# azrael417/mlperf-deepcam

Hardware: AMD Instinct MI355X
Metric: samples/sec (768x1152x16) train step (higher is better)
Workload: dtype bf16; 1 GPU; DeepLabV3+/Xception train step (fwd + weighted CE + bwd + LAMB), 768x1152x16, local_batch=8, bf16 activations / fp32 master weights, random-init seed 333; local_batch=8, global_batch=8, parallelism=dp1, optimizer=LAMB, hip_graph=False, launch_list_replay=False

## Files before the change

### mlperf-deepcam_amd/csrc/dwtile_s2.hip

```cpp
#include "dwtile.h"
#include "dwtile_common.h"
#include "mfma_tile.h"

namespace dc {

namespace {

static __device__ __attribute__((aligned(256))) unsigned char dws2_zero_page[256];

template <int CG, int TH_>
struct S2Cfg {
  static constexpr int TH = TH_, TW = 8 * (32 / CG);
  static constexpr int NSL = 128 / CG;
  static constexpr int SPR = TW / DT_PX;
  static constexpr int SPT = TH * SPR / NSL;
  static_assert(SPT * NSL == TH * SPR, "tile does not divide into strips");
};
constexpr int lds_bytes(int hh, int hw, int cg) { return (hh * hw * cg + 255) / 256 * 256 * 16; }

template <typename T, int HH, int HW, int CG>
__device__ inline void stage_tile(char* smem, const T* __restrict__ in, int ldin, int n, int iy0, int ix0, int cg0, int ngroups, int H,
                                  int W) {
  constexpr int KPV = Elem<T>::kPerVec;
  constexpr int HP = HH * HW, ITER = (HP * CG + 255) / 256;
  const int tid = threadIdx.x;
  const int wv = __builtin_amdgcn_readfirstlane(tid >> 6);
  const int g = tid % CG;
  const bool gok = cg0 + g < ngroups;
  const T* base = in + (size_t)n * H * W * ldin + (size_t)(cg0 + g) * KPV;
#pragma unroll
  for (int it = 0; it < ITER; ++it) {
    const int hp = (it * 256 + tid) / CG;
    const int hy = hp / HW, hx = hp - hy * HW;
    const int iy = iy0 + hy, ix = ix0 + hx;
    const bool ok = gok && hp < HP && (unsigned)iy < (unsigned)H && (unsigned)ix < (unsigned)W;
    const void* src = ok ? (const void*)(base + ((size_t)iy * W + ix) * ldin) : (const void*)dws2_zero_page;
    __builtin_amdgcn_global_load_lds((gas_ptr)src, (lds_ptr)(smem + (it * 256 + wv * 64) * 16), 16, 0, 0);
  }
}

struct S2Args {
  int Hi, Wi, Ho, Wo, C, ncgb, ntx, nty;
  const float* pscale;
  const float* pshift;
  int prelu;
};

template <typename T, int CG>
__global__ __launch_bounds__(256) void dws2_fwd_kernel(const T* __restrict__ in, int ldin, const float* __restrict__ wp,
                                                       T* __restrict__ out, int ldout, S2Args a) {
  typedef S2Cfg<CG, 4> K;
  constexpr int KPV = Elem<T>::kPerVec, KH = KPV / 2;
  constexpr int HH = 2 * K::TH + 1, HW = 2 * K::TW + 1, WC = 2 * DT_PX + 1;
  extern __shared__ __attribute__((aligned(16))) char smem[];
  const int t = xcd_remap(blockIdx.x, gridDim.x);
  const int cgb = t % a.ncgb;
  int r = t / a.ncgb;
  const int tx = r % a.ntx;
  r /= a.ntx;
  const int ty = r % a.nty, n = r / a.nty;
  const int ngroups = a.C / KPV;
  const int cg0 = cgb * CG, y0 = ty * K::TH, x0 = tx * K::TW;
  stage_tile<T, HH, HW, CG>(smem, in, ldin, n, 2 * y0 - 1, 2 * x0 - 1, cg0, ngroups, a.Hi, a.Wi);
  const int h = threadIdx.x % (2 * CG), sl = threadIdx.x / (2 * CG);
  const bool cok = cg0 + (h >> 1) < ngroups;
  const int ch0 = cok ? cg0 * KPV + h * KH : 0;
  float wk[9][KH];
  load_taps<KH>(wp, ch0, a.C, false, wk);
  __syncthreads();
  if (a.pscale != nullptr) {
    bn_transform_tile<T, HH, HW, CG>(smem, 2 * y0 - 1, 2 * x0 - 1, a.Hi, a.Wi, a.pscale, a.pshift, a.prelu, cg0, ngroups);
    __syncthreads();
  }
  if (!cok) return;
  const char* tile = smem + h * 8;
#pragma unroll 1
  for (int k = 0; k < K::SPT; ++k) {
    const int q = sl + K::NSL * k;
    const int row = q / K::SPR, xs = (q % K::SPR) * DT_PX;
    float acc[DT_PX][KH];
#pragma unroll
    for (int j = 0; j < DT_PX; ++j)
#pragma unroll
      for (int e = 0; e < KH; ++e) acc[j][e] = 0.f;
#pragma unroll
    for (int ky = 0; ky < 3; ++ky)
#pragma unroll
      for (int c = 0; c < WC; ++c) {
        float f[KH];
        unpack8(*reinterpret_cast<const vec8*>(tile + ((2 * row + ky) * HW + 2 * xs + c) * (CG * 16)), f, T());
#pragma unroll
        for (int kx = 0; kx < 3; ++kx) {
          if ((c - kx) >= 0 && ((c - kx) & 1) == 0 && (c - kx) / 2 < DT_PX) {
#pragma unroll
            for (int e = 0; e < KH; ++e) acc[(c - kx) / 2][e] = fmaf(f[e], wk[ky * 3 + kx][e], acc[(c - kx) / 2][e]);
          }
        }
      }
    const int oy = y0 + row;
    if (oy < a.Ho) {
#pragma unroll
      for (int j = 0; j < DT_PX; ++j) {
        const int ox = x0 + xs + j;
        if (ox < a.Wo) {
          vec8 v;
          pack8(v, acc[j], T());
          *reinterpret_cast<vec8*>(out + (((size_t)n * a.Ho + oy) * a.Wo + ox) * ldout + ch0) = v;
        }
      }
    }
  }
}

template <typename T, int CG, bool WG>
__global__ __launch_bounds__(256) void dws2_dgrad_kernel(const T* __restrict__ dy, int lddy, const float* __restrict__ wp,
                                                         const T* __restrict__ addend, int ldadd, T* __restrict__ dx, int lddx, S2Args a,
                                                         const DwBnStats st, int ntiles, int tpb) {
  typedef S2Cfg<CG, 8> K;
  constexpr int KPV = Elem<T>::kPerVec, KH = KPV / 2;
  constexpr int HH = K::TH / 2 + 1, HW = K::TW / 2 + 1;
  extern __shared__ __attribute__((aligned(16))) char smem[];
  const int t = xcd_remap(blockIdx.x, gridDim.x);
  const int cgb = t % a.ncgb;
  const int srow = t / a.ncgb;
  const int ngroups = a.C / KPV;
  const int cg0 = cgb * CG;
  const int h = threadIdx.x % (2 * CG), sl = threadIdx.x / (2 * CG);
  const bool cok = cg0 + (h >> 1) < ngroups;
  const int ch0 = cok ? cg0 * KPV + h * KH : 0;
  float wk[9][KH];
  load_taps<KH>(wp, ch0, a.C, false, wk);
  const bool stats = st.slab != nullptr;
  BnAcc<KH> bn;
  if (stats) bn.init(st, ch0);
  else if (WG) bn.init_affine(st, ch0);
  float dwa[WG ? 9 : 1][KH];
#pragma unroll
  for (int t9 = 0; t9 < (WG ? 9 : 1); ++t9)
#pragma unroll
    for (int e = 0; e < KH; ++e) dwa[t9][e] = 0.f;
  const char* tile = smem + h * 8;
  const int tbeg = srow * tpb, tend = min(ntiles, tbeg + tpb);
  for (int ti = tbeg; ti < tend; ++ti) {
    const int tx = ti % a.ntx;
    int r = ti / a.ntx;
    const int ty = r % a.nty, n = r / a.nty;
    const int y0 = ty * K::TH, x0 = tx * K::TW;
    if (ti != tbeg) __syncthreads();
    stage_tile<T, HH, HW, CG>(smem, dy, lddy, n, y0 / 2, x0 / 2, cg0, ngroups, a.Ho, a.Wo);
    auto load_y = [&](int k, vec8 (&yv)[DT_PX]) {
      const int q = sl + K::NSL * k;
      const int iy = y0 + q / K::SPR, xs = (q % K::SPR) * DT_PX;
#pragma unroll
      for (int j = 0; j < DT_PX; ++j) {
        const int ix = x0 + xs + j;
        vec8 z;
        z.w[0] = z.w[1] = 0u;
        yv[j] = (iy < a.Hi && ix < a.Wi) ? *reinterpret_cast<const vec8*>(reinterpret_cast<const T*>(st.y) + (((size_t)n * a.Hi + iy) * a.Wi + ix) * st.ldy + ch0) : z;
      }
    };
    vec8 yv[DT_PX], ynext[DT_PX];
    if (cok && (stats || WG)) load_y(0, yv);
    __syncthreads();
#pragma unroll 1
    for (int k = 0; k < (cok ? K::SPT : 0); ++k) {
      const int q = sl + K::NSL * k;
      const int row = q / K::SPR, xs = (q % K::SPR) * DT_PX;
      const int iy = y0 + row;
      if ((stats || WG) && k + 1 < K::SPT) load_y(k + 1, ynext);
      vec8 av[DT_PX];
      if (addend != nullptr) {
#pragma unroll
        for (int j = 0; j < DT_PX; ++j) {
          const int ix = x0 + xs + j;
          vec8 z;
          z.w[0] = z.w[1] = 0u;
          av[j] = (iy < a.Hi && ix < a.Wi) ? *reinterpret_cast<const vec8*>(addend + (((size_t)n * a.Hi + iy) * a.Wi + ix) * ldadd + ch0) : z;
        }
      }
      float acc[DT_PX][KH];
#pragma unroll
      for (int j = 0; j < DT_PX; ++j)
#pragma unroll
        for (int e = 0; e < KH; ++e) acc[j][e] = 0.f;
      float xh[WG ? DT_PX : 1][KH];
      if constexpr (WG) {
#pragma unroll
        for (int j = 0; j < DT_PX; ++j) {
          const bool in = iy < a.Hi && x0 + xs + j < a.Wi;
          float yf[KH];
          unpack8(yv[j], yf, T());
#pragma unroll
          for (int e = 0; e < KH; ++e) {
            const float v = fmaf(yf[e], bn.ms[e], bn.mh[e]);
            yf[e] = st.relu ? fmaxf(v, 0.f) : v;
          }
          vec8 rr;
          pack8(rr, yf, T());
          unpack8(rr, xh[j], T());
          if (!in) {
#pragma unroll
            for (int e = 0; e < KH; ++e) xh[j][e] = 0.f;
          }
        }
      }
#pragma unroll
      for (int ky = 0; ky < 3; ++ky) {
        const int num = row + 1 - ky;
        const bool yfit = (num & 1) == 0;
        const int trow = yfit ? num >> 1 : 0;
#pragma unroll
        for (int j = 0; j < DT_PX; ++j)
#pragma unroll
          for (int kx = 0; kx < 3; ++kx) {
            if (((j + 1 - kx) & 1) == 0) {
              const int tcol = (xs + j + 1 - kx) / 2;
              float f[KH];
              unpack8(*reinterpret_cast<const vec8*>(tile + (trow * HW + tcol) * (CG * 16)), f, T());
#pragma unroll
              for (int e = 0; e < KH; ++e) {
                const float fv = yfit ? f[e] : 0.f;
                acc[j][e] = fmaf(fv, wk[ky * 3 + kx][e], acc[j][e]);
                if constexpr (WG) dwa[ky * 3 + kx][e] = fmaf(fv, xh[j][e], dwa[ky * 3 + kx][e]);
              }
            }
          }
      }
      if (iy < a.Hi) {
#pragma unroll
        for (int j = 0; j < DT_PX; ++j) {
          const int ix = x0 + xs + j;
          if (ix < a.Wi) {
            if (addend != nullptr) {
              float ad[KH];
              unpack8(av[j], ad, T());
#pragma unroll
              for (int e = 0; e < KH; ++e) acc[j][e] += ad[e];
            }
            vec8 v;
            pack8(v, acc[j], T());
            *reinterpret_cast<vec8*>(dx + (((size_t)n * a.Hi + iy) * a.Wi + ix) * lddx + ch0) = v;
            if (stats) {
              float gs[KH], yf[KH];
              unpack8(v, gs, T());
              unpack8(yv[j], yf, T());
              bn.add(gs, yf, st.relu);
            }
          }
        }
      }
#pragma unroll
      for (int j = 0; j < DT_PX; ++j) yv[j] = ynext[j];
    }
  }
  if (stats) {
    __syncthreads();
    bn_acc_store<KH, K::NSL, CG * KPV>(reinterpret_cast<float*>(smem), bn.a, bn.b, cok, h, sl, st, srow, cg0 * KPV, a.C);
  }
  if constexpr (WG) {
    __syncthreads();
    float* red = reinterpret_cast<float*>(smem);
    constexpr int CW = CG * KPV;
    if (cok) {
#pragma unroll
      for (int tp = 0; tp < 9; ++tp)
#pragma unroll
        for (int e = 0; e < KH; ++e) red[(sl * 9 + tp) * CW + h * KH + e] = dwa[tp][e];
    }
    __syncthreads();
    for (int i = threadIdx.x; i < 9 * CW; i += 256) {
      const int tp = i / CW, cl = i % CW;
      const int c = cg0 * KPV + cl;
      if (c < a.C) {
        float s = 0.f;
#pragma unroll
        for (int q = 0; q < K::NSL; ++q) s += red[(q * 9 + tp) * CW + cl];
        st.wslab[((size_t)srow * 9 + tp) * a.C + c] = s;
      }
    }
  }
}

template <typename T, int CG>
__global__ __launch_bounds__(256) void dws2_wgrad_kernel(const T* __restrict__ x, int ldx, const T* __restrict__ dy, int lddy,
                                                         float* __restrict__ slab, S2Args a, int ntiles, int tpb) {
  typedef S2Cfg<CG, 4> K;
  constexpr int KPV = Elem<T>::kPerVec, KH = KPV / 2;
  constexpr int HH = 2 * K::TH + 1, HW = 2 * K::TW + 1, WC = 2 * DT_PX + 1;
  extern __shared__ __attribute__((aligned(16))) char smem[];
  const int t = xcd_remap(blockIdx.x, gridDim.x);
  const int cgb = t % a.ncgb, srow = t / a.ncgb;
  const int ngroups = a.C / KPV;
  const int cg0 = cgb * CG;
  const int h = threadIdx.x % (2 * CG), sl = threadIdx.x / (2 * CG);
  const bool cok = cg0 + (h >> 1) < ngroups;
  const int ch0 = cok ? cg0 * KPV + h * KH : 0;
  float acc[9][KH];
#pragma unroll
  for (int tp = 0; tp < 9; ++tp)
#pragma unroll
    for (int e = 0; e < KH; ++e) acc[tp][e] = 0.f;
  const int tbeg = srow * tpb, tend = min(ntiles, tbeg + tpb);
  const char* tile = smem + h * 8;
  for (int ti = tbeg; ti < tend; ++ti) {
    const int tx = ti % a.ntx;
    int r = ti / a.ntx;
    const int ty = r % a.nty, n = r / a.nty;
    const int y0 = ty * K::TH, x0 = tx * K::TW;
    if (ti != tbeg) __syncthreads();
    stage_tile<T, HH, HW, CG>(smem, x, ldx, n, 2 * y0 - 1, 2 * x0 - 1, cg0, ngroups, a.Hi, a.Wi);
    auto load_dy = [&](int k, vec8 (&gv)[DT_PX]) {
      const int q = sl + K::NSL * k;
      const int row = q / K::SPR, xs = (q % K::SPR) * DT_PX;
      const int oy = y0 + row;
#pragma unroll
      for (int j = 0; j < DT_PX; ++j) {
        const int ox = x0 + xs + j;
        const bool ok = cok && oy < a.Ho && ox < a.Wo;
        vec8 z;
        z.w[0] = z.w[1] = 0u;
        gv[j] = ok ? *reinterpret_cast<const vec8*>(dy + (((size_t)n * a.Ho + oy) * a.Wo + ox) * lddy + ch0) : z;
      }
    };
    vec8 gcur[DT_PX], gnext[DT_PX];
    load_dy(0, gcur);
    __syncthreads();
    if (a.pscale != nullptr) {
      bn_transform_tile<T, HH, HW, CG>(smem, 2 * y0 - 1, 2 * x0 - 1, a.Hi, a.Wi, a.pscale, a.pshift, a.prelu, cg0, ngroups);
      __syncthreads();
    }
    if (cok) {
#pragma unroll 1
      for (int k = 0; k < K::SPT; ++k) {
        if (k + 1 < K::SPT) load_dy(k + 1, gnext);
        const int q = sl + K::NSL * k;
        const int row = q / K::SPR, xs = (q % K::SPR) * DT_PX;
        float gf[DT_PX][KH];
#pragma unroll
        for (int j = 0; j < DT_PX; ++j) unpack8(gcur[j], gf[j], T());
#pragma unroll
        for (int ky = 0; ky < 3; ++ky)
#pragma unroll
          for (int c = 0; c < WC; ++c) {
            float f[KH];
            unpack8(*reinterpret_cast<const vec8*>(tile + ((2 * row + ky) * HW + 2 * xs + c) * (CG * 16)), f, T());
#pragma unroll
            for (int kx = 0; kx < 3; ++kx) {
              if ((c - kx) >= 0 && ((c - kx) & 1) == 0 && (c - kx) / 2 < DT_PX) {
#pragma unroll
                for (int e = 0; e < KH; ++e) acc[ky * 3 + kx][e] = fmaf(gf[(c - kx) / 2][e], f[e], acc[ky * 3 + kx][e]);
              }
            }
          }
#pragma unroll
        for (int j = 0; j < DT_PX; ++j) gcur[j] = gnext[j];
      }
    }
  }
  __syncthreads();
  float* red = reinterpret_cast<float*>(smem);
  constexpr int CW = CG * KPV;
#pragma unroll
  for (int tp = 0; tp < 9; ++tp)
#pragma unroll
    for (int e = 0; e < KH; ++e) red[(sl * 9 + tp) * CW + h * KH + e] = acc[tp][e];
  __syncthreads();
  for (int i = threadIdx.x; i < 9 * CW; i += 256) {
    const int tp = i / CW, cl = i % CW;
    const int c = cg0 * KPV + cl;
    if (c < a.C) {
      float s = 0.f;
#pragma unroll
      for (int q = 0; q < K::NSL; ++q) s += red[(q * 9 + tp) * CW + cl];
      slab[((size_t)srow * 9 + tp) * a.C + c] = s;
    }
  }
}

static int pick_cg(int ngroups) { return ngroups <= 8 ? 8 : ngroups <= 16 ? 16 : 32; }

constexpr int S2_DGRAD_WGS = 1024;
static int s2_dgrad_plan(int kpv, int C, int N, int Hi, int Wi, int* tpb_out) {
  const int cg = pick_cg(C / kpv);
  const int ntiles = N * cdiv(Hi, 8) * cdiv(Wi, 8 * (32 / cg));
  const int ncgb = cdiv(C / kpv, cg);
  int tpb = cdiv((long)ntiles * ncgb, S2_DGRAD_WGS);
  if (tpb < 1) tpb = 1;
  if (tpb_out) *tpb_out = tpb;
  return cdiv(ntiles, tpb);
}

template <typename T, int CG>
static void launch3(int mode, S2Args a, int N, const void* p0, int ld0, const float* wp, const void* p1, int ld1, void* out, int ldout,
                    float* slab, int* rows_out, hipStream_t st, DwBnStats bs) {
  constexpr int TW = 8 * (32 / CG);
  constexpr int LDS_F = lds_bytes(9, 2 * TW + 1, CG);
  constexpr int LDS_D0 = lds_bytes(5, TW / 2 + 1, CG);
  constexpr int FOLD2 = (128 / CG) * 2 * CG * Elem<T>::kPerVec * (int)sizeof(float);
  constexpr int LDS_D = LDS_D0 > FOLD2 ? LDS_D0 : FOLD2;
  constexpr int FOLD = (128 / CG) * 9 * CG * Elem<T>::kPerVec * (int)sizeof(float);
  a.ntx = cdiv(mode == 1 ? a.Wi : a.Wo, TW);
  a.nty = cdiv(mode == 1 ? a.Hi : a.Ho, mode == 1 ? 8 : 4);
  a.ncgb = cdiv(a.C / Elem<T>::kPerVec, CG);
  const int ntiles = N * a.ntx * a.nty;
  if (mode == 0) {
    DC_ONCE((void)hipFuncSetAttribute(reinterpret_cast<const void*>(&dws2_fwd_kernel<T, CG>), hipFuncAttributeMaxDynamicSharedMemorySize, LDS_F));
    hipLaunchKernelGGL((dws2_fwd_kernel<T, CG>), dim3(ntiles * a.ncgb), dim3(256), LDS_F, st, (const T*)p0, ld0, wp, (T*)out, ldout, a);
  } else if (mode == 1) {
    int tpb = 1;
    const int rows = s2_dgrad_plan(Elem<T>::kPerVec, a.C, N, a.Hi, a.Wi, &tpb);
    bs.rows = rows;
    if (rows_out) *rows_out = rows;
    if (bs.wslab != nullptr) {
      constexpr int LDS_DW = LDS_D > FOLD ? LDS_D : FOLD;
      DC_ONCE((void)hipFuncSetAttribute(reinterpret_cast<const void*>(&dws2_dgrad_kernel<T, CG, true>), hipFuncAttributeMaxDynamicSharedMemorySize, LDS_DW));
      hipLaunchKernelGGL((dws2_dgrad_kernel<T, CG, true>), dim3(rows * a.ncgb), dim3(256), LDS_DW, st, (const T*)p0, ld0, wp, (const T*)p1, ld1, (T*)out, ldout, a, bs, ntiles, tpb);
    } else {
      DC_ONCE((void)hipFuncSetAttribute(reinterpret_cast<const void*>(&dws2_dgrad_kernel<T, CG, false>), hipFuncAttributeMaxDynamicSharedMemorySize, LDS_D));
      hipLaunchKernelGGL((dws2_dgrad_kernel<T, CG, false>), dim3(rows * a.ncgb), dim3(256), LDS_D, st, (const T*)p0, ld0, wp, (const T*)p1, ld1, (T*)out, ldout, a, bs, ntiles, tpb);
    }
  } else {
    constexpr int LDS_W = LDS_F > FOLD ? LDS_F : FOLD;
    DC_ONCE((void)hipFuncSetAttribute(reinterpret_cast<const void*>(&dws2_wgrad_kernel<T, CG>), hipFuncAttributeMaxDynamicSharedMemorySize, LDS_W));
    long tpb = ((long)ntiles * a.ncgb + 256) / 512;
    if (tpb < 1) tpb = 1;
    while (cdiv(ntiles, tpb) > DWT_MAX_ROWS) ++tpb;
    const int rows = cdiv(ntiles, tpb);
    *rows_out = rows;
    hipLaunchKernelGGL((dws2_wgrad_kernel<T, CG>), dim3(rows * a.ncgb), dim3(256), LDS_W, st, (const T*)p0, ld0, (const T*)p1, ld1, slab, a, ntiles, (int)tpb);
  }
}

template <typename T>
static void launch2(int mode, const S2Args& a, int N, const void* p0, int ld0, const float* wp, const void* p1, int ld1, void* out,
                    int ldout, float* slab, int* rows_out, hipStream_t st, const DwBnStats& bs) {
  const int cg = pick_cg(a.C / Elem<T>::kPerVec);
  if (cg == 32) launch3<T, 32>(mode, a, N, p0, ld0, wp, p1, ld1, out, ldout, slab, rows_out, st, bs);
  else if (cg == 16) launch3<T, 16>(mode, a, N, p0, ld0, wp, p1, ld1, out, ldout, slab, rows_out, st, bs);
  else launch3<T, 8>(mode, a, N, p0, ld0, wp, p1, ld1, out, ldout, slab, rows_out, st, bs);
}

}

int launch_dw_tile_s2(int dtype, int mode, int N, int Hi, int Wi, int C, const void* p0, int ld0, const float* wp, const void* p1, int ld1,
                      void* out, int ldout, float* slab, int* rows_out, hipStream_t st, const float* pscale, const float* pshift, int prelu,
                      const DwBnStats* bnstats) {
  DwBnStats bs;
  if (bnstats != nullptr && mode == 1) bs = *bnstats; else { bs.slab = nullptr; bs.y = nullptr; bs.ldy = 0; bs.mean = bs.invstd = bs.mscale = bs.mshift = nullptr; bs.relu = 0; bs.rows = 0; bs.wslab = nullptr; }
  S2Args a;
  a.pscale = mode == 1 ? nullptr : pscale; a.pshift = pshift; a.prelu = prelu;
  a.Hi = Hi; a.Wi = Wi; a.Ho = (Hi - 1) / 2 + 1; a.Wo = (Wi - 1) / 2 + 1; a.C = C;
  a.ncgb = a.ntx = a.nty = 0;
  DC_REQUIRE((long)N * Hi * Wi < (1L << 31), "dc_dwconv: tensor too large for the tiled stride-2 path");
  int rows = 0;
  if (dtype == DC_BF16) launch2<bf16>(mode, a, N, p0, ld0, wp, p1, ld1, out, ldout, slab, &rows, st, bs);
  else launch2<float>(mode, a, N, p0, ld0, wp, p1, ld1, out, ldout, slab, &rows, st, bs);
  if (rows_out) *rows_out = rows;
  DC_LAUNCHED(mode == 0 ? "dw_tile_s2_fwd" : mode == 1 ? "dw_tile_s2_dgrad" : "dw_tile_s2_wgrad");
  return 0;
}

int dw_tile_s2_dgrad_rows(int dtype, int C, int N, int Hi, int Wi) { return s2_dgrad_plan(dtype == DC_BF16 ? 8 : 4, C, N, Hi, Wi, nullptr); }

}
```

Before: 269.8 samples/s.

## Double-buffer stride-2 depthwise dgrad tiles and specialize on row parity

```diff
diff --git a/mlperf-deepcam_amd/csrc/dwtile_s2.hip b/mlperf-deepcam_amd/csrc/dwtile_s2.hip
--- a/mlperf-deepcam_amd/csrc/dwtile_s2.hip
+++ b/mlperf-deepcam_amd/csrc/dwtile_s2.hip
@@ -112,13 +112,24 @@
   }
 }
 
-template <typename T, int CG, bool WG>
-__global__ __launch_bounds__(256) void dws2_dgrad_kernel(const T* __restrict__ dy, int lddy, const float* __restrict__ wp,
-                                                         const T* __restrict__ addend, int ldadd, T* __restrict__ dx, int lddx, S2Args a,
-                                                         const DwBnStats st, int ntiles, int tpb) {
+__device__ inline vec8 load8_if(const void* p, bool ok) {
+  vec8 v;
+  v.w[0] = v.w[1] = 0u;
+  if (ok) v = *reinterpret_cast<const vec8*>(p);
+  return v;
+}
+
+template <typename T, int CG, bool WG, bool ST>
+__global__ __launch_bounds__(256, 3) void dws2_dgrad_kernel(const T* __restrict__ dy, int lddy, const float* __restrict__ wp,
+                                                            const T* __restrict__ addend, int ldadd, T* __restrict__ dx, int lddx, S2Args a,
+                                                            const DwBnStats st, int ntiles, int tpb) {
   typedef S2Cfg<CG, 8> K;
   constexpr int KPV = Elem<T>::kPerVec, KH = KPV / 2;
   constexpr int HH = K::TH / 2 + 1, HW = K::TW / 2 + 1;
+  constexpr int TILE_B = lds_bytes(HH, HW, CG);
+  constexpr int RS = K::NSL / K::SPR;
+  static_assert(K::NSL % K::SPR == 0 && RS % 2 == 0, "the row parity of a thread's strips must not depend on the strip");
+  static_assert((2 * CG * K::SPR) % 64 == 0, "the row parity must be the same for the lanes of a wave");
   extern __shared__ __attribute__((aligned(16))) char smem[];
   const int t = xcd_remap(blockIdx.x, gridDim.x);
   const int cgb = t % a.ncgb;
@@ -128,118 +139,117 @@
   const int h = threadIdx.x % (2 * CG), sl = threadIdx.x / (2 * CG);
   const bool cok = cg0 + (h >> 1) < ngroups;
   const int ch0 = cok ? cg0 * KPV + h * KH : 0;
-  float wk[9][KH];
-  load_taps<KH>(wp, ch0, a.C, false, wk);
-  const bool stats = st.slab != nullptr;
+  const int r0 = sl / K::SPR, xs = (sl % K::SPR) * DT_PX;
+  const int par = __builtin_amdgcn_readfirstlane(r0 & 1);
+  constexpr bool stats = ST, needy = ST || WG;
+  const bool add = !ST && addend != nullptr;
   BnAcc<KH> bn;
   if (stats) bn.init(st, ch0);
   else if (WG) bn.init_affine(st, ch0);
-  float dwa[WG ? 9 : 1][KH];
-#pragma unroll
-  for (int t9 = 0; t9 < (WG ? 9 : 1); ++t9)
-#pragma unroll
-    for (int e = 0; e < KH; ++e) dwa[t9][e] = 0.f;
-  const char* tile = smem + h * 8;
+  float dwa[WG ? 6 : 1][KH];
+#pragma unroll
+  for (int t6 = 0; t6 < (WG ? 6 : 1); ++t6)
+#pragma unroll
+    for (int e = 0; e < KH; ++e) dwa[t6][e] = 0.f;
   const int tbeg = srow * tpb, tend = min(ntiles, tbeg + tpb);
-  for (int ti = tbeg; ti < tend; ++ti) {
-    const int tx = ti % a.ntx;
-    int r = ti / a.ntx;
-    const int ty = r % a.nty, n = r / a.nty;
-    const int y0 = ty * K::TH, x0 = tx * K::TW;
-    if (ti != tbeg) __syncthreads();
+
+  auto tiles = [&](auto par_tag) {
+    constexpr int PAR = decltype(par_tag)::value;
+    constexpr int NL = PAR ? 2 : 1;
+    float wl[3 * NL][KH];
+#pragma unroll
+    for (int l = 0; l < NL; ++l)
+#pragma unroll
+      for (int kx = 0; kx < 3; ++kx)
+#pragma unroll
+        for (int e = 0; e < KH; ++e) wl[l * 3 + kx][e] = wp[(size_t)((PAR ? 2 * l : 1) * 3 + kx) * a.C + ch0 + e];
+    auto coords = [&](int ti, int& n, int& y0, int& x0) {
+      const int r = ti / a.ntx;
+      x0 = (ti - r * a.ntx) * K::TW;
+      n = r / a.nty;
+      y0 = (r - n * a.nty) * K::TH;
+    };
+    auto pixel = [&](int n, int iy) { return ((unsigned)n * a.Hi + iy) * a.Wi; };
+    int n, y0, x0;
+    coords(tbeg, n, y0, x0);
     stage_tile<T, HH, HW, CG>(smem, dy, lddy, n, y0 / 2, x0 / 2, cg0, ngroups, a.Ho, a.Wo);
-    auto load_y = [&](int k, vec8 (&yv)[DT_PX]) {
-      const int q = sl + K::NSL * k;
-      const int iy = y0 + q / K::SPR, xs = (q % K::SPR) * DT_PX;
+    vec8 yv[DT_PX], av[DT_PX];
+    if (cok) {
+      const unsigned p = pixel(n, y0 + r0) + x0 + xs;
 #pragma unroll
       for (int j = 0; j < DT_PX; ++j) {
-        const int ix = x0 + xs + j;
-        vec8 z;
-        z.w[0] = z.w[1] = 0u;
-        yv[j] = (iy < a.Hi && ix < a.Wi) ? *reinterpret_cast<const vec8*>(reinterpret_cast<const T*>(st.y) + (((size_t)n * a.Hi + iy) * a.Wi + ix) * st.ldy + ch0) : z;
-      }
-    };
-    vec8 yv[DT_PX], ynext[DT_PX];
-    if (cok && (stats || WG)) load_y(0, yv);
-    __syncthreads();
+        const bool ok = y0 + r0 < a.Hi && x0 + xs + j < a.Wi;
+        if (needy) yv[j] = load8_if(reinterpret_cast<const T*>(st.y) + (size_t)(p + j) * st.ldy + ch0, ok);
+        if (add) av[j] = load8_if(addend + (size_t)(p + j) * ldadd + ch0, ok);
+      }
+    }
+    for (int ti = tbeg; ti < tend; ++ti) {
+      const char* tile = smem + ((ti - tbeg) & 1) * TILE_B + h * 8;
+      const bool more = ti + 1 < tend;
+      int nn = n, ny0 = y0, nx0 = x0;
+      if (more) coords(ti + 1, nn, ny0, nx0);
+      asm volatile("s_waitcnt vmcnt(0)" ::: "memory");
+      __syncthreads();
+      if (more) stage_tile<T, HH, HW, CG>(smem + ((ti + 1 - tbeg) & 1) * TILE_B, dy, lddy, nn, ny0 / 2, nx0 / 2, cg0, ngroups, a.Ho, a.Wo);
 #pragma unroll 1
-    for (int k = 0; k < (cok ? K::SPT : 0); ++k) {
-      const int q = sl + K::NSL * k;
-      const int row = q / K::SPR, xs = (q % K::SPR) * DT_PX;
-      const int iy = y0 + row;
-      if ((stats || WG) && k + 1 < K::SPT) load_y(k + 1, ynext);
-      vec8 av[DT_PX];
-      if (addend != nullptr) {
-#pragma unroll
-        for (int j = 0; j < DT_PX; ++j) {
-          const int ix = x0 + xs + j;
-          vec8 z;
-          z.w[0] = z.w[1] = 0u;
-          av[j] = (iy < a.Hi && ix < a.Wi) ? *reinterpret_cast<const vec8*>(addend + (((size_t)n * a.Hi + iy) * a.Wi + ix) * ldadd + ch0) : z;
-        }
-      }
-      float acc[DT_PX][KH];
-#pragma unroll
-      for (int j = 0; j < DT_PX; ++j)
-#pragma unroll
-        for (int e = 0; e < KH; ++e) acc[j][e] = 0.f;
-      float xh[WG ? DT_PX : 1][KH];
-      if constexpr (WG) {
+      for (int k = 0; k < (cok ? K::SPT : 0); ++k) {
+        const int row = r0 + RS * k;
+        const int iy = y0 + row;
+        const unsigned p = pixel(n, iy) + x0 + xs;
+        const bool last = k + 1 == K::SPT;
+        const int fy = last ? ny0 + r0 : iy + RS, fx = (last ? nx0 : x0) + xs;
+        const bool fok = (!last || more) && fy < a.Hi;
+        const unsigned fp = pixel(last ? nn : n, fy) + fx;
 #pragma unroll
         for (int j = 0; j < DT_PX; ++j) {
           const bool in = iy < a.Hi && x0 + xs + j < a.Wi;
-          float yf[KH];
-          unpack8(yv[j], yf, T());
-#pragma unroll
-          for (int e = 0; e < KH; ++e) {
-            const float v = fmaf(yf[e], bn.ms[e], bn.mh[e]);
-            yf[e] = st.relu ? fmaxf(v, 0.f) : v;
+          float xh[KH];
+          if constexpr (WG) {
+            float yf[KH];
+            unpack8(yv[j], yf, T());
+#pragma unroll
+            for (int e = 0; e < KH; ++e) {
+              const float v = fmaf(yf[e], bn.ms[e], bn.mh[e]);
+              yf[e] = st.relu ? fmaxf(v, 0.f) : v;
+            }
+            vec8 rr;
+            pack8(rr, yf, T());
+            unpack8(rr, xh, T());
+            if (!in) {
+#pragma unroll
+              for (int e = 0; e < KH; ++e) xh[e] = 0.f;
+            }
           }
-          vec8 rr;
-          pack8(rr, yf, T());
-          unpack8(rr, xh[j], T());
-          if (!in) {
-#pragma unroll
-            for (int e = 0; e < KH; ++e) xh[j][e] = 0.f;
+          float acc[KH];
+#pragma unroll
+          for (int e = 0; e < KH; ++e) acc[e] = 0.f;
+#pragma unroll
+          for (int l = 0; l < NL; ++l) {
+            const int trow = (row + 1 - (PAR ? 2 * l : 1)) >> 1;
+#pragma unroll
+            for (int kx = 0; kx < 3; ++kx) {
+              if (((j + 1 - kx) & 1) == 0) {
+                const int tcol = (xs + j + 1 - kx) / 2;
+                float f[KH];
+                unpack8(*reinterpret_cast<const vec8*>(tile + (trow * HW + tcol) * (CG * 16)), f, T());
+#pragma unroll
+                for (int e = 0; e < KH; ++e) {
+                  acc[e] = fmaf(f[e], wl[l * 3 + kx][e], acc[e]);
+                  if constexpr (WG) dwa[l * 3 + kx][e] = fmaf(f[e], xh[e], dwa[l * 3 + kx][e]);
+                }
+              }
+            }
           }
-        }
-      }
-#pragma unroll
-      for (int ky = 0; ky < 3; ++ky) {
-        const int num = row + 1 - ky;
-        const bool yfit = (num & 1) == 0;
-        const int trow = yfit ? num >> 1 : 0;
-#pragma unroll
-        for (int j = 0; j < DT_PX; ++j)
-#pragma unroll
-          for (int kx = 0; kx < 3; ++kx) {
-            if (((j + 1 - kx) & 1) == 0) {
-              const int tcol = (xs + j + 1 - kx) / 2;
-              float f[KH];
-              unpack8(*reinterpret_cast<const vec8*>(tile + (trow * HW + tcol) * (CG * 16)), f, T());
-#pragma unroll
-              for (int e = 0; e < KH; ++e) {
-                const float fv = yfit ? f[e] : 0.f;
-                acc[j][e] = fmaf(fv, wk[ky * 3 + kx][e], acc[j][e]);
-                if constexpr (WG) dwa[ky * 3 + kx][e] = fmaf(fv, xh[j][e], dwa[ky * 3 + kx][e]);
-              }
-            }
-          }
-      }
-      if (iy < a.Hi) {
-#pragma unroll
-        for (int j = 0; j < DT_PX; ++j) {
-          const int ix = x0 + xs + j;
-          if (ix < a.Wi) {
-            if (addend != nullptr) {
+          if (in) {
+            if (add) {
               float ad[KH];
               unpack8(av[j], ad, T());
 #pragma unroll
-              for (int e = 0; e < KH; ++e) acc[j][e] += ad[e];
+              for (int e = 0; e < KH; ++e) acc[e] += ad[e];
             }
             vec8 v;
-            pack8(v, acc[j], T());
-            *reinterpret_cast<vec8*>(dx + (((size_t)n * a.Hi + iy) * a.Wi + ix) * lddx + ch0) = v;
+            pack8(v, acc, T());
+            *reinterpret_cast<vec8*>(dx + (size_t)(p + j) * lddx + ch0) = v;
             if (stats) {
               float gs[KH], yf[KH];
               unpack8(v, gs, T());
@@ -247,12 +257,17 @@
               bn.add(gs, yf, st.relu);
             }
           }
+          const bool ok = fok && fx + j < a.Wi;
+          if (needy) yv[j] = load8_if(reinterpret_cast<const T*>(st.y) + (size_t)(fp + j) * st.ldy + ch0, ok);
+          if (add) av[j] = load8_if(addend + (size_t)(fp + j) * ldadd + ch0, ok);
         }
       }
-#pragma unroll
-      for (int j = 0; j < DT_PX; ++j) yv[j] = ynext[j];
-    }
-  }
+      n = nn; y0 = ny0; x0 = nx0;
+    }
+  };
+  if (par) tiles(std::integral_constant<int, 1>());
+  else tiles(std::integral_constant<int, 0>());
+
   if (stats) {
     __syncthreads();
     bn_acc_store<KH, K::NSL, CG * KPV>(reinterpret_cast<float*>(smem), bn.a, bn.b, cok, h, sl, st, srow, cg0 * KPV, a.C);
@@ -263,9 +278,11 @@
     constexpr int CW = CG * KPV;
     if (cok) {
 #pragma unroll
-      for (int tp = 0; tp < 9; ++tp)
-#pragma unroll
-        for (int e = 0; e < KH; ++e) red[(sl * 9 + tp) * CW + h * KH + e] = dwa[tp][e];
+      for (int tp = 0; tp < 9; ++tp) {
+        const int lo = tp < 3 ? tp : tp - 3;
+#pragma unroll
+        for (int e = 0; e < KH; ++e) red[(sl * 9 + tp) * CW + h * KH + e] = ((tp / 3 == 1) == (par == 0)) ? dwa[lo][e] : 0.f;
+      }
     }
     __syncthreads();
     for (int i = threadIdx.x; i < 9 * CW; i += 256) {
@@ -395,7 +412,7 @@
                     float* slab, int* rows_out, hipStream_t st, DwBnStats bs) {
   constexpr int TW = 8 * (32 / CG);
   constexpr int LDS_F = lds_bytes(9, 2 * TW + 1, CG);
-  constexpr int LDS_D0 = lds_bytes(5, TW / 2 + 1, CG);
+  constexpr int LDS_D0 = 2 * lds_bytes(5, TW / 2 + 1, CG);
   constexpr int FOLD2 = (128 / CG) * 2 * CG * Elem<T>::kPerVec * (int)sizeof(float);
   constexpr int LDS_D = LDS_D0 > FOLD2 ? LDS_D0 : FOLD2;
   constexpr int FOLD = (128 / CG) * 9 * CG * Elem<T>::kPerVec * (int)sizeof(float);
@@ -411,13 +428,19 @@
     const int rows = s2_dgrad_plan(Elem<T>::kPerVec, a.C, N, a.Hi, a.Wi, &tpb);
     bs.rows = rows;
     if (rows_out) *rows_out = rows;
+    constexpr int LDS_DW = LDS_D > FOLD ? LDS_D : FOLD;
+    auto go = [&](auto wg, auto stats) {
+      constexpr bool WG = decltype(wg)::value, ST = decltype(stats)::value;
+      constexpr int LDS = WG ? LDS_DW : LDS_D;
+      DC_ONCE((void)hipFuncSetAttribute(reinterpret_cast<const void*>(&dws2_dgrad_kernel<T, CG, WG, ST>), hipFuncAttributeMaxDynamicSharedMemorySize, LDS));
+      hipLaunchKernelGGL((dws2_dgrad_kernel<T, CG, WG, ST>), dim3(rows * a.ncgb), dim3(256), LDS, st, (const T*)p0, ld0, wp, (const T*)p1, ld1, (T*)out, ldout, a, bs, ntiles, tpb);
+    };
     if (bs.wslab != nullptr) {
-      constexpr int LDS_DW = LDS_D > FOLD ? LDS_D : FOLD;
-      DC_ONCE((void)hipFuncSetAttribute(reinterpret_cast<const void*>(&dws2_dgrad_kernel<T, CG, true>), hipFuncAttributeMaxDynamicSharedMemorySize, LDS_DW));
-      hipLaunchKernelGGL((dws2_dgrad_kernel<T, CG, true>), dim3(rows * a.ncgb), dim3(256), LDS_DW, st, (const T*)p0, ld0, wp, (const T*)p1, ld1, (T*)out, ldout, a, bs, ntiles, tpb);
+      if (bs.slab != nullptr) go(std::true_type(), std::true_type());
+      else go(std::true_type(), std::false_type());
     } else {
-      DC_ONCE((void)hipFuncSetAttribute(reinterpret_cast<const void*>(&dws2_dgrad_kernel<T, CG, false>), hipFuncAttributeMaxDynamicSharedMemorySize, LDS_D));
-      hipLaunchKernelGGL((dws2_dgrad_kernel<T, CG, false>), dim3(rows * a.ncgb), dim3(256), LDS_D, st, (const T*)p0, ld0, wp, (const T*)p1, ld1, (T*)out, ldout, a, bs, ntiles, tpb);
+      if (bs.slab != nullptr) go(std::false_type(), std::true_type());
+      else go(std::false_type(), std::false_type());
     }
   } else {
     constexpr int LDS_W = LDS_F > FOLD ? LDS_F : FOLD;
@@ -452,6 +475,7 @@
   a.Hi = Hi; a.Wi = Wi; a.Ho = (Hi - 1) / 2 + 1; a.Wo = (Wi - 1) / 2 + 1; a.C = C;
   a.ncgb = a.ntx = a.nty = 0;
   DC_REQUIRE((long)N * Hi * Wi < (1L << 31), "dc_dwconv: tensor too large for the tiled stride-2 path");
+  DC_REQUIRE(!(mode == 1 && bs.slab != nullptr && p1 != nullptr), "dc_dwconv: the stride-2 data gradient takes BatchNorm sums or an addend, not both");
   int rows = 0;
   if (dtype == DC_BF16) launch2<bf16>(mode, a, N, p0, ld0, wp, p1, ld1, out, ldout, slab, &rows, st, bs);
   else launch2<float>(mode, a, N, p0, ld0, wp, p1, ld1, out, ldout, slab, &rows, st, bs);
```

New measurement: 270.7 samples/s, median of 6. Within noise of the previous version (+0.3%).
